# wouter-rombouts/fast-losless-image-compression-format

Hardware: AMD Instinct MI355X
Metric: encode+decode MPixels/s on 4K RGBA at 1/2/4/8 MI355X; bitstream bit-exact (higher is better)
Workload: dtype u8

## Files before the change

### fast-losless-image-compression-format_amd/csrc/nice_dec_rec.hpp

```cpp
#pragma once
#include <hip/hip_runtime.h>
#include <stdint.h>

#include "nice_format.h"

namespace nice {

__device__ __forceinline__ void set_status(int32_t* st, int32_t code) {
  atomicCAS(reinterpret_cast<int*>(st), 0, code);
}

constexpr uint32_t REC_RUN = 1u << 28;
constexpr uint32_t REC_K = 0xFFu | (0xFFu << 10) | (0xFFu << 20);
constexpr uint32_t REC_TAG_MASK = (3u << 8) | (3u << 18);
__device__ __forceinline__ uint32_t rec_tagbits(uint32_t tag) { return ((tag & 3u) << 8) | ((tag >> 2) << 18); }
__device__ __forceinline__ uint32_t rec_canon(uint32_t r, uint32_t tag) {
  return (r & REC_TAG_MASK) == rec_tagbits(tag) ? r : REC_RUN;
}
__device__ __forceinline__ uint32_t rec_cls(uint32_t r) { return r >> 28; }
__device__ __forceinline__ uint32_t rec_c(uint32_t r) { return r & REC_K; }
__device__ __forceinline__ uint32_t rec_spread(uint32_t v) {
  return (v & 0xFFu) | ((v & 0xFF00u) << 2) | ((v & 0xFF0000u) << 4);
}
__host__ __device__ constexpr int cls_rows(int c) {
  return c < 4 ? 0 : c == 4 ? 1 : c == 5 ? 1 : c == 6 ? 2 : c == 7 ? 1 : c <= 10 ? 3 : c == 11 ? 1 : c <= 13 ? 3 : 0;
}
__host__ __device__ constexpr int cls_px(int c) {
  return c < 4 ? c : c == 4 ? 0 : c == 5 ? -1 : c == 6 ? 0 : c == 7 ? -3 : c == 8 ? -1 : c == 9 ? 0
       : c == 10 ? 1 : c == 11 ? 3 : c == 12 ? 3 : c == 13 ? -3 : 0;
}
__host__ __device__ constexpr int id_cls(int id) {
  return id == 0 ? 1 : id == 1 ? 4 : id == 2 ? 5 : id == 3 ? 2 : id == 4 ? 6
       : id == 5 ? 1 : id == 6 ? 4 : id == 7 ? 5 : id == 8 ? 7 : id == 9 ? 3 : id == 10 ? 8
       : id == 11 ? 9 : id == 12 ? 10 : id == 13 ? 11 : id == 14 ? 12 : 13;
}
__host__ __device__ constexpr bool cls_table_ok() {
  for (int id = 0; id < 16; ++id) {
    const int rows = id < 5 ? br_rows(id) : lr_rows(id - 5), px = id < 5 ? br_px(id) : lr_px(id - 5);
    if (cls_rows(id_cls(id)) != rows || cls_px(id_cls(id)) != px) return false;
  }
  return true;
}
static_assert(cls_table_ok(), "reference offsets (code.rs:141-145) map onto the record classes");
constexpr unsigned long long ID_CLS_PACK = [] {
  unsigned long long v = 0;
  for (int id = 0; id < 16; ++id) v |= (unsigned long long)id_cls(id) << (4 * id);
  return v;
}();
constexpr uint32_t CLS_ROWS_PACK = [] {
  uint32_t v = 0;
  for (int c = 0; c < 16; ++c) v |= (uint32_t)cls_rows(c) << (2 * c);
  return v;
}();
constexpr unsigned long long CLS_PX_PACK = [] {
  unsigned long long v = 0;
  for (int c = 0; c < 16; ++c) v |= (unsigned long long)(cls_px(c) + 3) << (3 * c);
  return v;
}();

}
```

### fast-losless-image-compression-format_amd/csrc/nice_decode.hip

```cpp
#include <hip/hip_runtime.h>
#include <stdint.h>

#include <type_traits>

#include "../../include/nice.h"
#include "nice_bits.hpp"
#include "nice_dec_rec.hpp"
#include "nice_format.h"
#include "nice_kernels.h"

namespace nice {

__device__ __forceinline__ uint32_t n_chunks(uint64_t len, uint64_t D, uint32_t cb) {
  const uint64_t bits = len * 8;
  return bits > D ? (uint32_t)((bits - D + cb - 1) / cb) : 0u;
}

__global__ __launch_bounds__(256) void dec_tables(DecArgs a) {
  __shared__ uint8_t lens[N_BINS];
  __shared__ uint8_t smax[N_STREAMS];
  __shared__ uint16_t order[N_BINS];
  __shared__ int bad;
  const uint32_t f = blockIdx.x;
  const uint64_t len = a.stream_len[f];
// ... 277 lines not shown
  uint4 pp[8];
};

__device__ inline void load_lut(LutLds& S, const DecTables* T) {
  const uint4* s = reinterpret_cast<const uint4*>(T->lut);
  uint4* d = reinterpret_cast<uint4*>(S.lut);
  for (uint32_t i = threadIdx.x; i < sizeof(S.lut) / 16; i += blockDim.x) d[i] = s[i];
  for (uint32_t i = threadIdx.x; i < N_BINS; i += blockDim.x) {
    S.lo[i] = T->lo[i];
    S.sym[i] = T->sym[i];
    S.len[i] = T->len[i];
  }
  if (threadIdx.x < N_STREAMS) {
    const int st = (int)threadIdx.x;
    S.gp[st] = (uint32_t)T->lut_off[st] | ((uint32_t)T->lut_bits[st] << 16) | ((uint32_t)T->max_aob[st] << 24);
    S.gs[st] = (uint32_t)stream_base(st) | ((uint32_t)stream_size(st) << 16);
  }
  if (threadIdx.x < 8u) {
    const uint32_t m = threadIdx.x;
    uint32_t w[4];
#pragma unroll
    for (uint32_t i = 0; i < 4; ++i) {
      const uint32_t st = m < 5u ? pay_stream(m, i) : 0u;
      w[i] = (32u - T->lut_bits[st]) | ((uint32_t)T->lut_off[st] << 17);
    }
    S.pp[m] = make_uint4(w[0], w[1], w[2], w[3]);
  }
}

__device__ __forceinline__ uint32_t stream_word(const uint8_t* p, uint64_t len, uint32_t w) {
  uint32_t v = 0;
  for (int k = 0; k < 4; ++k) {
    const uint64_t i = (uint64_t)w * 4 + k;
    v = (v << 8) | (i < len ? p[i] : (len ? p[len - 1] : 0u));
  }
  return v;
}

struct Lane {
  unsigned long long pos;
  unsigned long long win;
  uint32_t avail;
  uint32_t rp;
  uint32_t ws;
};
__device__ __forceinline__ bool lane_ok(const Lane& L) { return L.rp + PIXEL_WORDS <= RING_W; }

// ... 122 lines not shown
__device__ __forceinline__ uint32_t pixel_event_fast(Lane& L, const uint32_t* my, const LutLds& S,
                                                     const StreamParams& G, uint32_t& s0, uint32_t& s1,
                                                     uint32_t& s2, uint32_t& s3) {
  const uint32_t o = (uint32_t)(L.pos >> 5) - L.ws;
  const uint32_t sh = (uint32_t)L.pos & 31u;
  const uint32_t w0 = my[o], w1 = my[o + 1], w2 = my[o + 2];
  unsigned long long win = ((((unsigned long long)w0 << 32) | w1) << sh) | (((unsigned long long)w2 << sh) >> 32);
  uint32_t tot = 0;
  const uint32_t pfx = fsym(win, tot, S, G.g[PFX_STREAM]);
  if (pfx < (uint32_t)P_RUN1) {
    const bool rgb = pfx == (uint32_t)P_RGB, lu = pfx == (uint32_t)P_LUMA, l2 = pfx == (uint32_t)P_LUMA2;
    const uint4 pp = S.pp[pfx];
    s0 = fsym(win, tot, S, pp.x);
    if (rgb || lu || l2) {
      s1 = fsym(win, tot, S, pp.y);
      s2 = fsym(win, tot, S, pp.z);
      if (lu) s3 = fsym(win, tot, S, pp.w);
    }
  }
  L.pos += tot;
  return pfx;
}

__device__ __forceinline__ uint32_t pixel_event_fast_at(const uint32_t* my, const LutLds& S, uint32_t fp_pfx,
                                                        uint32_t o, uint32_t sh, uint32_t& s0, uint32_t& s1,
                                                        uint32_t& s2, uint32_t& s3, uint32_t& tot) {
  const uint32_t w0 = my[o], w1 = my[o + 1], w2 = my[o + 2];
  unsigned long long win = ((((unsigned long long)w0 << 32) | w1) << sh) | (((unsigned long long)w2 << sh) >> 32);
  tot = 0;
  const uint32_t pfx = fsym(win, tot, S, fp_pfx);
  if (pfx < (uint32_t)P_RUN1) {
    const bool rgb = pfx == (uint32_t)P_RGB, lu = pfx == (uint32_t)P_LUMA, l2 = pfx == (uint32_t)P_LUMA2;
    const uint4 pp = S.pp[pfx];
    s0 = fsym(win, tot, S, pp.x);
    if (rgb || lu || l2) {
      s1 = fsym(win, tot, S, pp.y);
      s2 = fsym(win, tot, S, pp.z);
      if (lu) s3 = fsym(win, tot, S, pp.w);
    }
  }
  return pfx;
}

__device__ __forceinline__ uint32_t pixel_count(uint32_t pfx, uint32_t& dk) {
  if (pfx < (uint32_t)P_RUN1) { dk = 0; return 1u; }
  const uint32_t sh = (3u * dk) & 63u;
  const uint64_t c = ((uint64_t)(pfx - P_RUN1) << sh) + (dk == 0 ? 1u : 0u);
  dk = dk >= 64u ? 1u : dk + 1u;
  return c > 0xFFFFFFFFull ? 0xFFFFFFFFu : (uint32_t)c;
}
__device__ __forceinline__ uint32_t sat_add(uint32_t a, uint32_t b) { return a + b < a ? 0xFFFFFFFFu : a + b; }

constexpr unsigned long long PS_MASK = (1ull << 51) - 1ull;
__device__ __forceinline__ unsigned long long ps_pack(unsigned long long rel, uint32_t dk) {
  return rel | ((unsigned long long)dk << 44);
}


__global__ __launch_bounds__(256) void dec_init_entries(DecArgs a) {
  const uint32_t f = blockIdx.y;
  for (uint32_t j = blockIdx.x * 256 + threadIdx.x; j < a.max_chunks; j += gridDim.x * 256) {
// ... 13 lines not shown

constexpr uint32_t SLICE_EMIT = 0, SLICE_HEAD_EMIT = 1, SLICE_PLACE = 2;
__device__ __forceinline__ uint32_t slice_route(const DecArgs& a, uint64_t base, uint32_t j, uint32_t& ag,
                                                uint32_t& nvalid, uint32_t& hn) {
  const unsigned long long last = a.last[base + j];
  ag = a.agree[base + j];
  const uint32_t nev = a.ev_n[base + j];
  unsigned long long e = 0;
  uint32_t hev_n = EV_OVERFLOW, hev_ag = AGREE_NONE;
  if (a.hev) {
    e = j == 0 ? 0ull : a.entry[base + j];
    hev_n = a.hev_n[base + j];
    hev_ag = a.hev_ag[base + j];
  }
  nvalid = (uint32_t)(last >> 56);
  hn = 0;
  if (ag == AGREE_NONE || nev == EV_OVERFLOW || ag > nvalid) return SLICE_EMIT;
  if (ag == 0u) return SLICE_PLACE;
  if ((last & PS_MASK) != e || hev_n == EV_OVERFLOW || hev_ag != ag) return SLICE_HEAD_EMIT;
  hn = hev_n;
  return SLICE_PLACE;
}

__device__ __forceinline__ uint32_t ev_pack(uint32_t pfx, uint32_t s0, uint32_t s1, uint32_t s2, uint32_t s3) {
  return pfx | (s0 << 3) | (s1 << 12) | (s2 << 20) | (pfx == (uint32_t)P_LUMA ? s3 << 7 : 0u);
}

__global__ __launch_bounds__(DEC_PARSE_THREADS) PARSE_ATTR void dec_sync(DecArgs a, uint32_t* changed, const uint32_t* prev,
                                                              uint32_t* fchanged) {
  __shared__ LutLds S;
  __shared__ __attribute__((aligned(16))) uint32_t ring[DEC_PARSE_THREADS * RING_STRIDE];
  if (prev && *prev == 0) return;
  const uint32_t f = blockIdx.x / a.chunk_blocks;
  const uint32_t jb = blockIdx.x % a.chunk_blocks;
  if (a.status[f] != 0) return;
  const uint64_t len = a.stream_len[f];
  const uint64_t D = a.data_start[f];
  const uint32_t nc = n_chunks(len, D, a.chunk_bits);
  if (jb * DEC_PARSE_THREADS >= nc) return;
  const uint32_t j = jb * DEC_PARSE_THREADS + threadIdx.x;
  const uint64_t base = (uint64_t)f * a.max_chunks;
  unsigned long long e = 0, last = ~0ull;
  if (j < nc) {
    e = j == 0 ? 0ull : a.entry[base + j];
    last = a.last[base + j];
  }
  const bool need = j < nc && (last == ~0ull || (last & PS_MASK) != e);
  if (!__syncthreads_or(need)) return;
  load_lut(S, reinterpret_cast<const DecTables*>(a.tables) + f);
// ... 100 lines not shown
      constexpr bool HEAD = decltype(keep_tag)::value == 2;
      if (active && (r >= rlim || px > N)) active = false;
      if (active && r >= nck) {
        const uint32_t cur = (r - b31) | (dk << 20);
        if (check && k < nvalid_old && (uint32_t)ck_old == cur) {
          synced = true;
          active = false;
        } else {
          ck[(uint64_t)k * a.max_chunks] = cur | ((unsigned long long)px << 32);
          if (keep) evck[(uint64_t)k * a.max_chunks] = ne;
          ++k;
          nck = k < a.n_ck ? nck + a.ck_bits : 0xFFFFFFFFu;
          ck_old = (check && k < nvalid_old) ? ck[(uint64_t)k * a.max_chunks] : ~0ull;
        }
      }
      if ((!(KEEP || HEAD) || SLOT == 0) && !__any(active)) return false;
      if (__any(active && r >= rfill)) {
        const uint32_t wsa = (bwl + (r >> 5)) & ~3u;
        ring_fill_ws(wring, p, len, al16, wsa);
        wsr = wsa - bwl;
        rfill = (wsr + RING_W - 2u) << 5;
      }
      if (active) {
        uint32_t s0 = 0, s1 = 0, s2 = 0, s3 = 0, tot;
        const uint32_t pfx = pixel_event_fast_at(my, S, fp_pfx, (r >> 5) - wsr, r & 31u, s0, s1, s2, s3, tot);
        r += tot;
        uint32_t c;
        if (pfx < (uint32_t)P_RUN1) {
          dk = 0;
          c = 1u;
        } else {
          const uint32_t sh = (3u * dk) & 63u, d = pfx - (uint32_t)P_RUN1;
          if (sh < 30u) {
            c = (d << sh) + (dk == 0 ? 1u : 0u);
          } else {
            const uint64_t c64 = (uint64_t)d << sh;
            c = c64 > 0xFFFFFFFFull ? 0xFFFFFFFFu : (uint32_t)c64;
          }
          dk = dk >= 64u ? 1u : dk + 1u;
        }
        px = sat_add(px, c);
        if (KEEP && keep) {
          const uint32_t ev = pfx < (uint32_t)P_RUN1 ? ev_pack(pfx, s0, s1, s2, s3) : EV_RUN | min(c, EV_RUN - 1u);
          if constexpr (SLOT == 0) q0 = ev;
          if constexpr (SLOT == 1) q1 = ev;
          if constexpr (SLOT == 2) q2 = ev;
          if constexpr (SLOT == 3) {
            q3 = ev;
            if (ne < a.ev_cap) *reinterpret_cast<uint4*>(evp + ev_word(ne - 3u)) = make_uint4(q0, q1, q2, q3);
          }
          ++ne;
        }
        if (HEAD && hkeep) {
          const uint32_t ev = pfx < (uint32_t)P_RUN1 ? ev_pack(pfx, s0, s1, s2, s3) : EV_RUN | min(c, EV_RUN - 1u);
          if constexpr (SLOT == 0) q0 = ev;
          if constexpr (SLOT == 1) q1 = ev;
          if constexpr (SLOT == 2) q2 = ev;
          if constexpr (SLOT == 3) {
            q3 = ev;
            if (ne < a.hev_cap) *reinterpret_cast<uint4*>(evp + ev_word(ne - 3u)) = make_uint4(q0, q1, q2, q3);
          }
          ++ne;
        }
      }
      return true;
    };
    using keep_none = std::integral_constant<int, 0>;
    using keep_first = std::integral_constant<int, 1>;
    using keep_head = std::integral_constant<int, 2>;
    if (__any(keep && active)) {
      for (;;) {
        if (!step(std::integral_constant<int, 0>{}, keep_first{})) break;
        if (!step(std::integral_constant<int, 1>{}, keep_first{})) break;
        if (!step(std::integral_constant<int, 2>{}, keep_first{})) break;
        if (!step(std::integral_constant<int, 3>{}, keep_first{})) break;
      }
    } else if (__any(hkeep && active)) {
// ... 288 lines not shown
      if (dk != 0 && pfx == (uint32_t)P_RUN1) (void)pixel_count(pfx, dk);
      else active = false;
      continue;
    }
    if (pfx < (uint32_t)P_RUN1) {
      (void)rd(pay_stream(pfx, 0));
      if (pfx == (uint32_t)P_RGB || pfx == (uint32_t)P_LUMA || pfx == (uint32_t)P_LUMA2) {
        (void)rd(pay_stream(pfx, 1));
        (void)rd(pay_stream(pfx, 2));
        if (pfx == (uint32_t)P_LUMA) (void)rd(S_LUMA_OTHER);
      }
      q += 1;
      dk = 0;
      closed = false;
    } else {
      q += pixel_count(pfx, dk);
      closed = closed || q == N;
    }
  }
  if (hang) set_status(&a.status[f], NICE_E_UNSUPPORTED);
}


__device__ __forceinline__ uint32_t make_event_rec(uint64_t W, uint32_t mode, uint32_t s0, uint32_t s1,
                                                   uint32_t s2, uint32_t s3) {
  const bool isbr = mode == P_BACK_REF, islu = mode == P_LUMA;
  const bool issd = mode == P_SMALL_DIFF, isl2 = mode == P_LUMA2;
  const uint32_t id = min(isbr ? s0 : 5u + s0, 15u);
  const uint32_t cls = (uint32_t)(ID_CLS_PACK >> (4 * id)) & 15u;
  const uint64_t rows = (CLS_ROWS_PACK >> (2 * cls)) & 3u;
  const int64_t off = (int64_t)(rows * W) + (int64_t)((CLS_PX_PACK >> (3 * cls)) & 7u) - 3;
  const bool bad0 = (isbr && s0 >= 5u) || (islu && s0 >= 11u) || off < 0;
  const uint32_t gl = (s1 - 32u) & 255u;
  const uint32_t c_lu = ((s2 - 16u + gl) & 255u) | (gl << 10) | (((s3 - 16u + gl) & 255u) << 20);
  const uint32_t rd = s0 % 7u, t1 = s0 / 7u;
  const uint32_t c_sd = ((rd - 3u) & 255u) | ((((t1 % 7u) - 3u) & 255u) << 10) | ((((t1 / 7u) - 3u) & 255u) << 20);
  const uint32_t g2 = (s0 - 32u) & 255u;
  const uint32_t c_l2 = ((s1 - 16u + g2) & 255u) | (g2 << 10) | (((s2 - 16u + g2) & 255u) << 20);
  const uint32_t c_rgb = (s0 & 255u) | ((s1 & 255u) << 10) | ((s2 & 255u) << 20);
  const uint32_t r = (isbr || islu) ? ((cls << 28) | (islu ? c_lu : 0u)) : issd ? c_sd : isl2 ? c_l2 : c_rgb;
  return r | (isl2 ? EV_L2 : 0u) | ((isbr || islu) && bad0 ? EV_BAD : 0u);
}
__device__ __forceinline__ bool rec_bad_at(uint32_t ev, uint64_t q, uint64_t W) {
  const uint32_t cls = rec_cls(ev);
  const uint64_t rows = (CLS_ROWS_PACK >> (2 * cls)) & 3u;
  const uint64_t off = rows * W + ((CLS_PX_PACK >> (3 * cls)) & 7u) - 3u;
  return (ev & EV_BAD) || ((ev & EV_L2) ? q < W : (cls != 0u && q < off));
}
__device__ __forceinline__ uint32_t make_record(uint64_t W, uint64_t q, uint32_t mode, uint32_t s0,
                                                uint32_t s1, uint32_t s2, uint32_t s3, bool& bad) {
  const uint32_t ev = make_event_rec(W, mode, s0, s1, s2, s3);
  bad = rec_bad_at(ev, q, W);
  return ev & ~(EV_L2 | EV_BAD);
}

struct RecGroup {
  unsigned long long grp;
  uint32_t v0, v1, v2, v3, mask;
  __device__ __forceinline__ void flush(uint32_t* rec, unsigned long long lo, unsigned long long hi) {
    if (!mask) return;
    if (grp >= lo && grp + 4 <= hi) {
      uint4* dst = reinterpret_cast<uint4*>(__builtin_assume_aligned(rec + grp, 16));
      *dst = make_uint4(v0, v1, v2, v3);
    } else {
      if (mask & 1u) rec[grp] = v0;
      if (mask & 2u) rec[grp + 1] = v1;
      if (mask & 4u) rec[grp + 2] = v2;
      if (mask & 8u) rec[grp + 3] = v3;
    }
  }
  __device__ __forceinline__ void put(uint32_t* rec, unsigned long long lo, unsigned long long cur,
                                      uint32_t r) {
    const unsigned long long g4 = cur & ~3ull;
    if (g4 != grp) {
      flush(rec, lo, cur);
      grp = g4;
      v0 = v1 = v2 = v3 = REC_RUN;
// ... 179 lines not shown
    if (route == SLICE_EMIT) return min(subs, 1u + nvalid / step);
    if (route == SLICE_PLACE) return 0u;
    return (ag + step - 1) / step;
  };
  uint32_t cnt = 0;
  for (uint32_t j = c0; j < c1; ++j) cnt += nsub(j);
  part[threadIdx.x] = cnt;
  __syncthreads();
  for (uint32_t d = 1; d < 1024; d <<= 1) {
    const uint32_t t = threadIdx.x >= d ? part[threadIdx.x - d] : 0u;
    __syncthreads();
    part[threadIdx.x] += t;
    __syncthreads();
  }
  uint32_t o = part[threadIdx.x] - cnt;
  uint32_t* items = a.head_items + base * subs;
  for (uint32_t j = c0; j < c1; ++j) {
    const uint32_t n = nsub(j);
    for (uint32_t s = 0; s < n; ++s) items[o++] = j * subs + s;
  }
  if (threadIdx.x == 1023) a.head_count[f] = part[1023];
}

__device__ __forceinline__ uint32_t place_record(uint32_t ev, uint32_t q, uint32_t W, const uint32_t* sdl,
                                                 const uint2* idt, bool& bad) {
  const uint32_t pfx = ev & 7u;
  const uint32_t pm = 1u << pfx;
  const bool isbr = (pm & (1u << P_BACK_REF)) != 0u, islu = (pm & (1u << P_LUMA)) != 0u;
  const bool issd = (pm & (1u << P_SMALL_DIFF)) != 0u, isl2 = (pm & (1u << P_LUMA2)) != 0u;
  const uint32_t s0 = (ev >> 3) & 511u, s1 = (ev >> 12) & 255u, s2 = (ev >> 20) & 255u, s3 = (ev >> 7) & 31u;
  const uint32_t s0l = s0 & 15u;
  const uint32_t id = min(isbr ? s0 : 5u + s0l, 15u);
  const uint2 ct = idt[id];
  const uint32_t cls = ct.x, off3 = ct.y;
  const bool bad_ref = (isbr && s0 >= 5u) || (islu && s0l >= 11u) || off3 < 3u || q + 3u < off3;
  const uint32_t gl = (s1 - 32u) & 255u;
  const uint32_t c_lu = ((s2 - 16u + gl) & 255u) | (gl << 10) | (((s3 - 16u + gl) & 255u) << 20);
  const uint32_t c_sd = sdl[min(s0, 342u)];
  const uint32_t g2 = (s0 - 32u) & 255u;
  const uint32_t c_l2 = ((s1 - 16u + g2) & 255u) | (g2 << 10) | (((s2 - 16u + g2) & 255u) << 20);
  uint32_t c_rgb = (s0 & 255u) | (s1 << 10) | (s2 << 20);
  bad = (isbr || islu) ? bad_ref : (isl2 && q < W);
  uint32_t c_br = (cls << 28) | (islu ? c_lu : 0u);
  uint32_t c_sd2 = c_sd, c_l22 = c_l2;
  asm volatile("" : "+v"(c_br), "+v"(c_sd2), "+v"(c_l22), "+v"(c_rgb));
  return (isbr || islu) ? c_br : issd ? c_sd2 : isl2 ? c_l22 : c_rgb;
}

struct alignas(16) SdlTable {
  uint32_t v[344];
};
constexpr SdlTable make_sdl_table() {
  SdlTable t{};
  for (uint32_t i = 0; i < 343u; ++i) {
    const uint32_t rd = i % 7u, t1 = i / 7u;
    t.v[i] = ((rd - 3u) & 255u) | ((((t1 % 7u) - 3u) & 255u) << 10) | ((((t1 / 7u) - 3u) & 255u) << 20);
  }
  return t;
}
__device__ __constant__ SdlTable kSdl = make_sdl_table();

__global__ __launch_bounds__(64 * DEC_PLACE_WAVES) void dec_place(DecArgs a) {
  __shared__ __attribute__((aligned(16))) uint32_t sdl[344];
  __shared__ uint2 idt[16];
  if (threadIdx.x < 16u) {
    const uint32_t id = threadIdx.x;
    const uint32_t cls = (uint32_t)(ID_CLS_PACK >> (4u * id)) & 15u;
    idt[id] = make_uint2(cls, (uint32_t)((CLS_ROWS_PACK >> (2u * cls)) & 3u) * a.W +
                                  (uint32_t)((CLS_PX_PACK >> (3u * cls)) & 7u));
  }
  if (threadIdx.x < 86u)
    reinterpret_cast<uint4*>(sdl)[threadIdx.x] = reinterpret_cast<const uint4*>(kSdl.v)[threadIdx.x];
  __syncthreads();
  const uint32_t lane = threadIdx.x & 63u;
  const uint32_t nbx = gridDim.x, nwg = nbx * gridDim.y, lin = blockIdx.y * nbx + blockIdx.x;
  const uint32_t xq = nwg / 8u, xr = nwg % 8u, xcd = lin % 8u;
  const uint32_t lg = (xcd < xr ? xcd * (xq + 1u) : xr * (xq + 1u) + (xcd - xr) * xq) + lin / 8u;
  const uint32_t f = lg / nbx, j = (lg % nbx) * DEC_PLACE_WAVES + (uint32_t)__builtin_amdgcn_readfirstlane((int)(threadIdx.x >> 6));
  if (a.status[f] != 0) return;
  const uint64_t len = a.stream_len[f];
  const uint64_t D = a.data_start[f];
  if (j >= n_chunks(len, D, a.chunk_bits)) return;
  const uint64_t base = (uint64_t)f * a.max_chunks;
  uint32_t ag, nvalid, hn;
  const uint32_t route = slice_route(a, base, j, ag, nvalid, hn);
  const uint32_t nev = a.ev_n[base + j];
  if (a.stats && lane == 0) {
    const uint32_t b = nev == EV_OVERFLOW ? 7u : ag == AGREE_NONE ? 6u : ag == 0u ? 0u : ag == 1u ? 1u
                     : ag <= 4u ? 2u : ag <= 16u ? 3u : ag <= 64u ? 4u : 5u;
    atomicAdd(&a.stats[50 + b], 1ull);
    atomicAdd(&a.stats[route == SLICE_EMIT ? 29 : route == SLICE_HEAD_EMIT ? 28 : ag == 0u ? 26 : 27], 1ull);
  }
  if (route == SLICE_EMIT) return;
  const bool head = route == SLICE_PLACE && ag != 0u;
  const uint64_t cki = (uint64_t)f * a.n_ck * a.max_chunks + j + (uint64_t)(ag ? ag - 1u : 0u) * a.max_chunks;
  auto uni = [](uint32_t v) { return (uint32_t)__builtin_amdgcn_readfirstlane((int)v); };
  const uint32_t i_first1 = uni(ag == 0u ? 0u : a.ev_ck[cki]), nev1 = uni(nev);
  hn = uni(hn);
  const unsigned long long q_first = a.chunk_start[base + j];
  const unsigned long long q_meet_v = q_first + (ag == 0u ? 0ull : (a.ck[cki] >> 32));
  const unsigned long long q_meet = ((unsigned long long)uni((uint32_t)(q_meet_v >> 32)) << 32) | uni((uint32_t)q_meet_v);
  unsigned long long q = head ? q_first : q_meet;
  const uint64_t N = (uint64_t)a.W * a.H;
  if (q > N) return;
  uint32_t* rec = a.recs + (uint64_t)f * a.rec_stride;
  const bool strict = (a.flags & NICE_DEC_STRICT_REFERENCE) != 0;
  bool err = false, stopped = false;
  for (uint32_t part = head ? 0u : 1u; part < 2u && !stopped; ++part) {
  const uint32_t* evp = part == 0u ? a.hev + hev_group(a, f, j) : a.ev + ev_group(a, f, j);
  const uint32_t i_first = part == 0u ? 0u : i_first1, nev = part == 0u ? hn : nev1;
  if (part == 1u && head && q != q_meet) {
    if (lane == 0) {
      if (a.stats) atomicAdd(&a.stats[30], 1ull);
      set_status(&a.status[f], NICE_E_HIP);
    }
    return;
  }
  if (i_first >= nev) continue;
  const uint32_t ev_last = nev - 1u;
  uint32_t nx[4];
#pragma unroll
  for (int k = 0; k < 4; ++k) nx[k] = evp[ev_word(min(i_first + 64u * k + lane, ev_last))];
  for (uint32_t i = i_first; i < nev; i += 256u) {
    uint32_t ev[4], r[4];
#pragma unroll
    for (int k = 0; k < 4; ++k) {
      ev[k] = nx[k];
      nx[k] = evp[ev_word(min(i + 256u + 64u * k + lane, ev_last))];
    }
    {
      const uint32_t N32 = (uint32_t)N;
      uint32_t c32[4];
      bool big = false;
#pragma unroll
      for (int k = 0; k < 4; ++k) {
        const bool valid = i + 64u * k + lane < nev;
        c32[k] = valid ? ((ev[k] & EV_RUN) ? (ev[k] & ~EV_RUN) : 1u) : 0u;
        big = big || c32[k] >= 65536u;
      }
      if (!__any(big)) {
        uint32_t qb[4];
        uint32_t base = (uint32_t)q;
        bool stop = false;
#pragma unroll
        for (int k = 0; k < 4; ++k) {
          if (i + 64u * k >= nev) break;
          const bool valid = i + 64u * k + lane < nev;
          const bool run = (ev[k] & EV_RUN) != 0u;
          const uint32_t incl = wave_incl_scan(c32[k]);
          qb[k] = base + incl - c32[k];
          base += (uint32_t)__builtin_amdgcn_readlane((int)incl, 63);
          bool rbad = false;
          r[k] = place_record(ev[k], min(qb[k], N32), a.W, sdl, idt, rbad);
          stop = stop || (valid && (qb[k] >= N32 || (run ? qb[k] + c32[k] > N32 : rbad)));
        }
        if (!__any(stop)) {
#pragma unroll
          for (int k = 0; k < 4; ++k) {
            if (i + 64u * k >= nev) break;
            if (i + 64u * k + lane < nev && !(ev[k] & EV_RUN)) rec[qb[k]] = r[k] | rec_tagbits(a.rec_tag);
          }
          q = base;
          continue;
        }
      }
    }
    unsigned long long c[4], qk[4], carry = 0;
    uint32_t stop_k = 4u, stop_lane = 64u;
    bool stop_at_n = false, stop_run = false;
#pragma unroll
    for (int k = 0; k < 4; ++k) {
      const uint32_t x = i + 64u * k + lane;
      const bool valid = x < nev;
      const bool run = (ev[k] & EV_RUN) != 0u;
      c[k] = valid ? (run ? (ev[k] & ~EV_RUN) : 1u) : 0u;
      unsigned long long incl;
      if (!__any(c[k] >= (1u << 25))) {
        incl = wave_incl_scan((uint32_t)c[k]);
      } else {
        incl = c[k];
#pragma unroll
        for (int o = 1; o < 64; o <<= 1) {
          const unsigned long long t = __shfl_up(incl, o);
          if ((int)lane >= o) incl += t;
        }
      }
      const unsigned long long qb = q + carry + incl - c[k];
      carry += __shfl(incl, 63);
      qk[k] = qb;
      bool rbad = false;
      r[k] = place_record(ev[k], (uint32_t)min(qb, N), a.W, sdl, idt, rbad);
      const bool at_n = valid && qb == N && !(run && c[k] == 0);
      const bool bad = valid && !at_n && (run ? qb + c[k] > N : rbad);
      const unsigned long long m = __ballot(at_n || bad);
      if (stop_k == 4u && m) {
        stop_k = (uint32_t)k;
        stop_lane = (uint32_t)__builtin_ctzll(m);
        stop_at_n = __shfl(at_n ? 1 : 0, (int)stop_lane) != 0;
        stop_run = __shfl(run ? 1 : 0, (int)stop_lane) != 0;
      }
    }
#pragma unroll
    for (int k = 0; k < 4; ++k) {
      const bool keep = (uint32_t)k < stop_k || ((uint32_t)k == stop_k && lane < stop_lane);
      if (keep && i + 64u * k + lane < nev && !(ev[k] & EV_RUN)) rec[qk[k]] = r[k] | rec_tagbits(a.rec_tag);
    }
    if (stop_k < 4u) {
      if (lane == 0) err = stop_at_n ? (strict && stop_run) : true;
      stopped = true;
      break;
    }
    q += carry;
  }
  }
// ... 6 lines not shown
```

### fast-losless-image-compression-format_amd/csrc/nice_kernels.h

```cpp
#pragma once
#include <hip/hip_runtime.h>
#include <stdint.h>

#include "nice_geom.h"

namespace nice {

constexpr uint32_t FLAG_LONG = 1u;
constexpr uint32_t FLAG_BAD = 2u;

struct EncArgs {
  const uint8_t* px;
  uint64_t frame_stride;
  uint32_t n_frames, W, H, C;
  uint8_t channels_out;
  uint32_t tiles_per_frame, tiles_per_block;
  uint8_t* out;
  uint64_t out_stride;
  unsigned long long* out_len;
  uint32_t* hist;
  uint32_t* tile_first;
  uint32_t* tile_last;
  uint32_t* tile_next;
  uint32_t* cmask;
// ... 114 lines not shown
  uint32_t* ev_n;
  uint32_t* agree;
  uint32_t* head_items;
  uint32_t* head_count;
  uint32_t* hev;
  uint32_t hev_cap;
  uint32_t* hev_n;
  uint32_t* hev_ag;
  uint32_t strips;
  unsigned long long* hand;
  uint32_t* hand_abort;
  uint32_t split_f0;
  uint32_t redo;
  uint32_t test_absent_strip;
  uint32_t flow_k, flow_ring;
  const uint32_t* unsettled;
  const unsigned long long* stream_off;
  uint64_t packed_bytes;
};
__device__ __forceinline__ const uint8_t* dec_stream_ptr(const DecArgs& a, uint32_t f) {
  return a.streams + (a.stream_off ? (uint64_t)a.stream_off[f] : (uint64_t)f * a.stream_stride);
}
constexpr uint32_t SPLIT_ABORT_ERR = 1u, SPLIT_REDO = 2u;
constexpr uint32_t EV_RUN = 1u << 31, EV_BAD = 1u << 9, EV_L2 = 1u << 8;
constexpr uint32_t EV_OVERFLOW = 0xFFFFFFFFu, AGREE_NONE = 0xFFFFu;

__global__ void dec_tables(DecArgs a);
__global__ void dec_init_entries(DecArgs a);
__global__ void dec_sync(DecArgs a, uint32_t* changed, const uint32_t* prev, uint32_t* fchanged);
__global__ void dec_sync_settle(DecArgs a, const uint32_t* last_changed, const uint32_t* fchanged, uint32_t* settled);
__global__ void dec_scan(DecArgs a);
__global__ void dec_strict_refill(DecArgs a);
__global__ void dec_emit(DecArgs a);
__global__ void dec_place(DecArgs a);
__global__ void dec_heads(DecArgs a);
__global__ void dec_reconstruct(DecArgs a);
__global__ void dec_rows(DecArgs a);
__global__ void dec_rows_wide(DecArgs a);
__global__ void dec_rows8(DecArgs a);
__global__ void dec_rows_flow(DecArgs a);
__global__ void dec_rows_split(DecArgs a);

__device__ __forceinline__ uint32_t wave_incl_scan(uint32_t v) {
  v += (uint32_t)__builtin_amdgcn_update_dpp(0, (int)v, 0x111, 0xF, 0xF, false);
  v += (uint32_t)__builtin_amdgcn_update_dpp(0, (int)v, 0x112, 0xF, 0xF, false);
  v += (uint32_t)__builtin_amdgcn_update_dpp(0, (int)v, 0x114, 0xF, 0xF, false);
  v += (uint32_t)__builtin_amdgcn_update_dpp(0, (int)v, 0x118, 0xF, 0xF, false);
// ... 14 lines not shown
```

Before: 69290.

## Repack decode events so placement becomes table-driven masked ORs

Changes the event word layout so each decoded symbol is shifted into its final record bit position during parsing, using shifts stored in the per-prefix LUT entry. Placement then builds a record from a 128-entry shared table of class/mask entries plus a small-diff lookup, replacing per-event branch-heavy reconstruction. A deep-region fast path skips the per-event reference bounds check once the position is at least three rows in. This cuts ALU work in dec_place at the cost of larger shared tables and a new event encoding shared between parse and place, which must stay consistent.

```diff
diff --git a/fast-losless-image-compression-format_amd/csrc/nice_dec_event.hpp b/fast-losless-image-compression-format_amd/csrc/nice_dec_event.hpp
--- /dev/null
+++ b/fast-losless-image-compression-format_amd/csrc/nice_dec_event.hpp
@@ -0,0 +1,164 @@
+#pragma once
+#include <stdint.h>
+
+#include "nice_format.h"
+
+#ifndef NICE_HDI
+#if defined(__HIPCC__) || defined(__CUDACC__)
+#define NICE_HDI __host__ __device__ __forceinline__
+#else
+#define NICE_HDI inline
+#endif
+#endif
+
+namespace nice {
+
+constexpr uint32_t REC_RUN = 1u << 28;
+constexpr uint32_t REC_K = 0xFFu | (0xFFu << 10) | (0xFFu << 20);
+constexpr uint32_t REC_TAG_MASK = (3u << 8) | (3u << 18);
+NICE_HDI uint32_t rec_tagbits(uint32_t tag) { return ((tag & 3u) << 8) | ((tag >> 2) << 18); }
+NICE_HDI uint32_t rec_canon(uint32_t r, uint32_t tag) {
+  return (r & REC_TAG_MASK) == rec_tagbits(tag) ? r : REC_RUN;
+}
+NICE_HDI uint32_t rec_cls(uint32_t r) { return r >> 28; }
+NICE_HDI uint32_t rec_c(uint32_t r) { return r & REC_K; }
+NICE_HDI uint32_t rec_spread(uint32_t v) {
+  return (v & 0xFFu) | ((v & 0xFF00u) << 2) | ((v & 0xFF0000u) << 4);
+}
+NICE_HD constexpr int cls_rows(int c) {
+  return c < 4 ? 0 : c == 4 ? 1 : c == 5 ? 1 : c == 6 ? 2 : c == 7 ? 1 : c <= 10 ? 3 : c == 11 ? 1 : c <= 13 ? 3 : 0;
+}
+NICE_HD constexpr int cls_px(int c) {
+  return c < 4 ? c : c == 4 ? 0 : c == 5 ? -1 : c == 6 ? 0 : c == 7 ? -3 : c == 8 ? -1 : c == 9 ? 0
+       : c == 10 ? 1 : c == 11 ? 3 : c == 12 ? 3 : c == 13 ? -3 : 0;
+}
+NICE_HD constexpr int id_cls(int id) {
+  return id == 0 ? 1 : id == 1 ? 4 : id == 2 ? 5 : id == 3 ? 2 : id == 4 ? 6
+       : id == 5 ? 1 : id == 6 ? 4 : id == 7 ? 5 : id == 8 ? 7 : id == 9 ? 3 : id == 10 ? 8
+       : id == 11 ? 9 : id == 12 ? 10 : id == 13 ? 11 : id == 14 ? 12 : 13;
+}
+NICE_HD constexpr bool cls_table_ok() {
+  for (int id = 0; id < 16; ++id) {
+    const int rows = id < 5 ? br_rows(id) : lr_rows(id - 5), px = id < 5 ? br_px(id) : lr_px(id - 5);
+    if (cls_rows(id_cls(id)) != rows || cls_px(id_cls(id)) != px) return false;
+  }
+  return true;
+}
+static_assert(cls_table_ok(), "reference offsets (code.rs:141-145) map onto the record classes");
+constexpr unsigned long long ID_CLS_PACK = [] {
+  unsigned long long v = 0;
+  for (int id = 0; id < 16; ++id) v |= (unsigned long long)id_cls(id) << (4 * id);
+  return v;
+}();
+constexpr uint32_t CLS_ROWS_PACK = [] {
+  uint32_t v = 0;
+  for (int c = 0; c < 16; ++c) v |= (uint32_t)cls_rows(c) << (2 * c);
+  return v;
+}();
+constexpr unsigned long long CLS_PX_PACK = [] {
+  unsigned long long v = 0;
+  for (int c = 0; c < 16; ++c) v |= (unsigned long long)(cls_px(c) + 3) << (3 * c);
+  return v;
+}();
+
+constexpr uint32_t EV_BAD = 1u << 9, EV_L2 = 1u << 8;
+
+NICE_HDI uint32_t make_event_rec(uint64_t W, uint32_t mode, uint32_t s0, uint32_t s1, uint32_t s2, uint32_t s3) {
+  const bool isbr = mode == P_BACK_REF, islu = mode == P_LUMA;
+  const bool issd = mode == P_SMALL_DIFF, isl2 = mode == P_LUMA2;
+  const uint32_t idr = isbr ? s0 : 5u + s0;
+  const uint32_t id = idr < 15u ? idr : 15u;
+  const uint32_t cls = (uint32_t)(ID_CLS_PACK >> (4 * id)) & 15u;
+  const uint64_t rows = (CLS_ROWS_PACK >> (2 * cls)) & 3u;
+  const int64_t off = (int64_t)(rows * W) + (int64_t)((CLS_PX_PACK >> (3 * cls)) & 7u) - 3;
+  const bool bad0 = (isbr && s0 >= 5u) || (islu && s0 >= 11u) || off < 0;
+  const uint32_t gl = (s1 - 32u) & 255u;
+  const uint32_t c_lu = ((s2 - 16u + gl) & 255u) | (gl << 10) | (((s3 - 16u + gl) & 255u) << 20);
+  const uint32_t rd = s0 % 7u, t1 = s0 / 7u;
+  const uint32_t c_sd = ((rd - 3u) & 255u) | ((((t1 % 7u) - 3u) & 255u) << 10) | ((((t1 / 7u) - 3u) & 255u) << 20);
+  const uint32_t g2 = (s0 - 32u) & 255u;
+  const uint32_t c_l2 = ((s1 - 16u + g2) & 255u) | (g2 << 10) | (((s2 - 16u + g2) & 255u) << 20);
+  const uint32_t c_rgb = (s0 & 255u) | ((s1 & 255u) << 10) | ((s2 & 255u) << 20);
+  const uint32_t r = (isbr || islu) ? ((cls << 28) | (islu ? c_lu : 0u)) : issd ? c_sd : isl2 ? c_l2 : c_rgb;
+  return r | (isl2 ? EV_L2 : 0u) | ((isbr || islu) && bad0 ? EV_BAD : 0u);
+}
+NICE_HDI bool rec_bad_at(uint32_t ev, uint64_t q, uint64_t W) {
+  const uint32_t cls = rec_cls(ev);
+  const uint64_t rows = (CLS_ROWS_PACK >> (2 * cls)) & 3u;
+  const uint64_t off = rows * W + ((CLS_PX_PACK >> (3 * cls)) & 7u) - 3u;
+  return (ev & EV_BAD) || ((ev & EV_L2) ? q < W : (cls != 0u && q < off));
+}
+NICE_HDI uint32_t make_record(uint64_t W, uint64_t q, uint32_t mode, uint32_t s0, uint32_t s1, uint32_t s2,
+                              uint32_t s3, bool& bad) {
+  const uint32_t ev = make_event_rec(W, mode, s0, s1, s2, s3);
+  bad = rec_bad_at(ev, q, W);
+  return ev & ~(EV_L2 | EV_BAD);
+}
+
+constexpr uint32_t EV_RUN = 1u << 31;
+constexpr uint32_t EV_PFX_SHIFT = 28, EV_ID_SHIFT = 16;
+NICE_HD constexpr uint32_t ev_shift(uint32_t pfx, uint32_t i) {
+  return pfx == (uint32_t)P_BACK_REF ? (i == 0 ? EV_ID_SHIFT : 0u)
+       : pfx == (uint32_t)P_RGB ? (i == 0 ? 0u : i == 1 ? 10u : i == 2 ? 20u : 0u)
+       : pfx == (uint32_t)P_LUMA ? (i == 0 ? EV_ID_SHIFT : i == 1 ? 10u : i == 2 ? 0u : 20u)
+       : pfx == (uint32_t)P_LUMA2 ? (i == 0 ? 10u : i == 1 ? 0u : i == 2 ? 20u : 0u)
+       : 0u;
+}
+NICE_HDI uint32_t ev_pack(uint32_t pfx, uint32_t s0, uint32_t s1, uint32_t s2, uint32_t s3) {
+  return (pfx << EV_PFX_SHIFT) | (s0 << ev_shift(pfx, 0)) | (s1 << ev_shift(pfx, 1)) | (s2 << ev_shift(pfx, 2)) |
+         (s3 << ev_shift(pfx, 3));
+}
+
+struct alignas(16) PlaceEnt {
+  uint32_t cls, ml, mr, msd;
+};
+constexpr uint32_t PLACE_ENTRIES = 128;
+NICE_HDI PlaceEnt place_entry(uint32_t entry, uint32_t W, uint32_t& off3) {
+  const uint32_t pfx = entry & 7u, idf = entry >> 3;
+  const bool isbr = pfx == (uint32_t)P_BACK_REF, islu = pfx == (uint32_t)P_LUMA;
+  const bool isl2 = pfx == (uint32_t)P_LUMA2;
+  const uint32_t idr = isbr ? idf : 5u + idf;
+  const uint32_t id = idr < 15u ? idr : 15u;
+  const uint32_t cls = (uint32_t)(ID_CLS_PACK >> (4u * id)) & 15u;
+  const uint32_t o3 = (uint32_t)((CLS_ROWS_PACK >> (2u * cls)) & 3u) * W + (uint32_t)((CLS_PX_PACK >> (3u * cls)) & 7u);
+  const bool rejected = (isbr && idf >= 5u) || (islu && idf >= 11u) || o3 < 3u;
+  const bool isref = isbr || islu;
+  off3 = isref ? (rejected ? 0xFFFFFFFFu : o3) : isl2 ? W + 3u : 0u;
+  PlaceEnt e;
+  e.cls = isref ? cls << 28 : 0u;
+  e.ml = (islu || isl2) ? REC_K : 0u;
+  e.mr = pfx == (uint32_t)P_RGB ? REC_K : (isref && rejected) ? EV_BAD : 0u;
+  e.msd = pfx == (uint32_t)P_SMALL_DIFF ? 511u : 0u;
+  return e;
+}
+struct alignas(16) SdlTable {
+  uint32_t v[344];
+};
+constexpr SdlTable make_sdl_table() {
+  SdlTable t{};
+  for (uint32_t i = 0; i < 343u; ++i) {
+    const uint32_t rd = i % 7u, t1 = i / 7u;
+    t.v[i] = ((rd - 3u) & 255u) | ((((t1 % 7u) - 3u) & 255u) << 10) | ((((t1 / 7u) - 3u) & 255u) << 20);
+  }
+  return t;
+}
+
+constexpr uint32_t EV_LUMA_MASK = 0xFFu | (0x3Fu << 10) | (0xFFu << 20);
+constexpr uint32_t EV_LUMA_K = 240u | (224u << 10) | (240u << 20);
+
+NICE_HDI bool place_deep(uint64_t q0, uint64_t W) { return q0 >= 3u * W + 3u; }
+
+template <bool CHECK>
+NICE_HDI uint32_t place_record(uint32_t ev, uint32_t q, const uint32_t* sdl, const PlaceEnt* idt,
+                               const uint32_t* off3, bool& bad) {
+  const uint32_t entry = ((ev >> (EV_ID_SHIFT - 3u)) & 0x78u) | (ev >> EV_PFX_SHIFT);
+  const PlaceEnt t = idt[entry];
+  const uint32_t c_sd = sdl[(ev & t.msd) | (343u & ~t.msd)];
+  const uint32_t lt = (ev & EV_LUMA_MASK) + EV_LUMA_K;
+  const uint32_t x = lt + ((lt >> 10) & 255u) * 0x100001u;
+  if (CHECK) bad = q + 3u < off3[entry];
+  else bad = t.mr == EV_BAD;
+  return t.cls | (x & t.ml) | (ev & t.mr) | c_sd;
+}
+
+}
diff --git a/fast-losless-image-compression-format_amd/csrc/nice_dec_rec.hpp b/fast-losless-image-compression-format_amd/csrc/nice_dec_rec.hpp
--- a/fast-losless-image-compression-format_amd/csrc/nice_dec_rec.hpp
+++ b/fast-losless-image-compression-format_amd/csrc/nice_dec_rec.hpp
@@ -2,6 +2,7 @@
 #include <hip/hip_runtime.h>
 #include <stdint.h>
 
+#include "nice_dec_event.hpp"
 #include "nice_format.h"
 
 namespace nice {
@@ -10,52 +11,4 @@
   atomicCAS(reinterpret_cast<int*>(st), 0, code);
 }
 
-constexpr uint32_t REC_RUN = 1u << 28;
-constexpr uint32_t REC_K = 0xFFu | (0xFFu << 10) | (0xFFu << 20);
-constexpr uint32_t REC_TAG_MASK = (3u << 8) | (3u << 18);
-__device__ __forceinline__ uint32_t rec_tagbits(uint32_t tag) { return ((tag & 3u) << 8) | ((tag >> 2) << 18); }
-__device__ __forceinline__ uint32_t rec_canon(uint32_t r, uint32_t tag) {
-  return (r & REC_TAG_MASK) == rec_tagbits(tag) ? r : REC_RUN;
 }
-__device__ __forceinline__ uint32_t rec_cls(uint32_t r) { return r >> 28; }
-__device__ __forceinline__ uint32_t rec_c(uint32_t r) { return r & REC_K; }
-__device__ __forceinline__ uint32_t rec_spread(uint32_t v) {
-  return (v & 0xFFu) | ((v & 0xFF00u) << 2) | ((v & 0xFF0000u) << 4);
-}
-__host__ __device__ constexpr int cls_rows(int c) {
-  return c < 4 ? 0 : c == 4 ? 1 : c == 5 ? 1 : c == 6 ? 2 : c == 7 ? 1 : c <= 10 ? 3 : c == 11 ? 1 : c <= 13 ? 3 : 0;
-}
-__host__ __device__ constexpr int cls_px(int c) {
-  return c < 4 ? c : c == 4 ? 0 : c == 5 ? -1 : c == 6 ? 0 : c == 7 ? -3 : c == 8 ? -1 : c == 9 ? 0
-       : c == 10 ? 1 : c == 11 ? 3 : c == 12 ? 3 : c == 13 ? -3 : 0;
-}
-__host__ __device__ constexpr int id_cls(int id) {
-  return id == 0 ? 1 : id == 1 ? 4 : id == 2 ? 5 : id == 3 ? 2 : id == 4 ? 6
-       : id == 5 ? 1 : id == 6 ? 4 : id == 7 ? 5 : id == 8 ? 7 : id == 9 ? 3 : id == 10 ? 8
-       : id == 11 ? 9 : id == 12 ? 10 : id == 13 ? 11 : id == 14 ? 12 : 13;
-}
-__host__ __device__ constexpr bool cls_table_ok() {
-  for (int id = 0; id < 16; ++id) {
-    const int rows = id < 5 ? br_rows(id) : lr_rows(id - 5), px = id < 5 ? br_px(id) : lr_px(id - 5);
-    if (cls_rows(id_cls(id)) != rows || cls_px(id_cls(id)) != px) return false;
-  }
-  return true;
-}
-static_assert(cls_table_ok(), "reference offsets (code.rs:141-145) map onto the record classes");
-constexpr unsigned long long ID_CLS_PACK = [] {
-  unsigned long long v = 0;
-  for (int id = 0; id < 16; ++id) v |= (unsigned long long)id_cls(id) << (4 * id);
-  return v;
-}();
-constexpr uint32_t CLS_ROWS_PACK = [] {
-  uint32_t v = 0;
-  for (int c = 0; c < 16; ++c) v |= (uint32_t)cls_rows(c) << (2 * c);
-  return v;
-}();
-constexpr unsigned long long CLS_PX_PACK = [] {
-  unsigned long long v = 0;
-  for (int c = 0; c < 16; ++c) v |= (unsigned long long)(cls_px(c) + 3) << (3 * c);
-  return v;
-}();
-
-}
diff --git a/fast-losless-image-compression-format_amd/csrc/nice_decode.hip b/fast-losless-image-compression-format_amd/csrc/nice_decode.hip
--- a/fast-losless-image-compression-format_amd/csrc/nice_decode.hip
+++ b/fast-losless-image-compression-format_amd/csrc/nice_decode.hip
@@ -323,7 +323,7 @@
 #pragma unroll
     for (uint32_t i = 0; i < 4; ++i) {
       const uint32_t st = m < 5u ? pay_stream(m, i) : 0u;
-      w[i] = (32u - T->lut_bits[st]) | ((uint32_t)T->lut_off[st] << 17);
+      w[i] = (32u - T->lut_bits[st]) | (ev_shift(m, i) << 5) | ((uint32_t)T->lut_off[st] << 17);
     }
     S.pp[m] = make_uint4(w[0], w[1], w[2], w[3]);
   }
@@ -492,9 +492,11 @@
   return pfx;
 }
 
+template <bool EV = false>
 __device__ __forceinline__ uint32_t pixel_event_fast_at(const uint32_t* my, const LutLds& S, uint32_t fp_pfx,
                                                         uint32_t o, uint32_t sh, uint32_t& s0, uint32_t& s1,
-                                                        uint32_t& s2, uint32_t& s3, uint32_t& tot) {
+                                                        uint32_t& s2, uint32_t& s3, uint32_t& tot,
+                                                        uint32_t* evw = nullptr) {
   const uint32_t w0 = my[o], w1 = my[o + 1], w2 = my[o + 2];
   unsigned long long win = ((((unsigned long long)w0 << 32) | w1) << sh) | (((unsigned long long)w2 << sh) >> 32);
   tot = 0;
@@ -503,10 +505,15 @@
     const bool rgb = pfx == (uint32_t)P_RGB, lu = pfx == (uint32_t)P_LUMA, l2 = pfx == (uint32_t)P_LUMA2;
     const uint4 pp = S.pp[pfx];
     s0 = fsym(win, tot, S, pp.x);
+    if constexpr (EV) *evw = (pfx << EV_PFX_SHIFT) | (s0 << ((pp.x >> 5) & 31u));
     if (rgb || lu || l2) {
       s1 = fsym(win, tot, S, pp.y);
       s2 = fsym(win, tot, S, pp.z);
-      if (lu) s3 = fsym(win, tot, S, pp.w);
+      if constexpr (EV) *evw |= (s1 << ((pp.y >> 5) & 31u)) | (s2 << ((pp.z >> 5) & 31u));
+      if (lu) {
+        s3 = fsym(win, tot, S, pp.w);
+        if constexpr (EV) *evw |= s3 << ((pp.w >> 5) & 31u);
+      }
     }
   }
   return pfx;
@@ -566,9 +573,6 @@
   return SLICE_PLACE;
 }
 
-__device__ __forceinline__ uint32_t ev_pack(uint32_t pfx, uint32_t s0, uint32_t s1, uint32_t s2, uint32_t s3) {
-  return pfx | (s0 << 3) | (s1 << 12) | (s2 << 20) | (pfx == (uint32_t)P_LUMA ? s3 << 7 : 0u);
-}
 
 __global__ __launch_bounds__(DEC_PARSE_THREADS) PARSE_ATTR void dec_sync(DecArgs a, uint32_t* changed, const uint32_t* prev,
                                                               uint32_t* fchanged) {
@@ -715,8 +719,9 @@
         rfill = (wsr + RING_W - 2u) << 5;
       }
       if (active) {
-        uint32_t s0 = 0, s1 = 0, s2 = 0, s3 = 0, tot;
-        const uint32_t pfx = pixel_event_fast_at(my, S, fp_pfx, (r >> 5) - wsr, r & 31u, s0, s1, s2, s3, tot);
+        uint32_t s0 = 0, s1 = 0, s2 = 0, s3 = 0, tot, evw = 0;
+        const uint32_t pfx = pixel_event_fast_at<KEEP || HEAD>(my, S, fp_pfx, (r >> 5) - wsr, r & 31u, s0, s1, s2,
+                                                               s3, tot, &evw);
         r += tot;
         uint32_t c;
         if (pfx < (uint32_t)P_RUN1) {
@@ -734,7 +739,7 @@
         }
         px = sat_add(px, c);
         if (KEEP && keep) {
-          const uint32_t ev = pfx < (uint32_t)P_RUN1 ? ev_pack(pfx, s0, s1, s2, s3) : EV_RUN | min(c, EV_RUN - 1u);
+          const uint32_t ev = pfx < (uint32_t)P_RUN1 ? evw : EV_RUN | min(c, EV_RUN - 1u);
           if constexpr (SLOT == 0) q0 = ev;
           if constexpr (SLOT == 1) q1 = ev;
           if constexpr (SLOT == 2) q2 = ev;
@@ -745,7 +750,7 @@
           ++ne;
         }
         if (HEAD && hkeep) {
-          const uint32_t ev = pfx < (uint32_t)P_RUN1 ? ev_pack(pfx, s0, s1, s2, s3) : EV_RUN | min(c, EV_RUN - 1u);
+          const uint32_t ev = pfx < (uint32_t)P_RUN1 ? evw : EV_RUN | min(c, EV_RUN - 1u);
           if constexpr (SLOT == 0) q0 = ev;
           if constexpr (SLOT == 1) q1 = ev;
           if constexpr (SLOT == 2) q2 = ev;
@@ -1080,37 +1085,6 @@
 }
 
 
-__device__ __forceinline__ uint32_t make_event_rec(uint64_t W, uint32_t mode, uint32_t s0, uint32_t s1,
-                                                   uint32_t s2, uint32_t s3) {
-  const bool isbr = mode == P_BACK_REF, islu = mode == P_LUMA;
-  const bool issd = mode == P_SMALL_DIFF, isl2 = mode == P_LUMA2;
-  const uint32_t id = min(isbr ? s0 : 5u + s0, 15u);
-  const uint32_t cls = (uint32_t)(ID_CLS_PACK >> (4 * id)) & 15u;
-  const uint64_t rows = (CLS_ROWS_PACK >> (2 * cls)) & 3u;
-  const int64_t off = (int64_t)(rows * W) + (int64_t)((CLS_PX_PACK >> (3 * cls)) & 7u) - 3;
-  const bool bad0 = (isbr && s0 >= 5u) || (islu && s0 >= 11u) || off < 0;
-  const uint32_t gl = (s1 - 32u) & 255u;
-  const uint32_t c_lu = ((s2 - 16u + gl) & 255u) | (gl << 10) | (((s3 - 16u + gl) & 255u) << 20);
-  const uint32_t rd = s0 % 7u, t1 = s0 / 7u;
-  const uint32_t c_sd = ((rd - 3u) & 255u) | ((((t1 % 7u) - 3u) & 255u) << 10) | ((((t1 / 7u) - 3u) & 255u) << 20);
-  const uint32_t g2 = (s0 - 32u) & 255u;
-  const uint32_t c_l2 = ((s1 - 16u + g2) & 255u) | (g2 << 10) | (((s2 - 16u + g2) & 255u) << 20);
-  const uint32_t c_rgb = (s0 & 255u) | ((s1 & 255u) << 10) | ((s2 & 255u) << 20);
-  const uint32_t r = (isbr || islu) ? ((cls << 28) | (islu ? c_lu : 0u)) : issd ? c_sd : isl2 ? c_l2 : c_rgb;
-  return r | (isl2 ? EV_L2 : 0u) | ((isbr || islu) && bad0 ? EV_BAD : 0u);
-}
-__device__ __forceinline__ bool rec_bad_at(uint32_t ev, uint64_t q, uint64_t W) {
-  const uint32_t cls = rec_cls(ev);
-  const uint64_t rows = (CLS_ROWS_PACK >> (2 * cls)) & 3u;
-  const uint64_t off = rows * W + ((CLS_PX_PACK >> (3 * cls)) & 7u) - 3u;
-  return (ev & EV_BAD) || ((ev & EV_L2) ? q < W : (cls != 0u && q < off));
-}
-__device__ __forceinline__ uint32_t make_record(uint64_t W, uint64_t q, uint32_t mode, uint32_t s0,
-                                                uint32_t s1, uint32_t s2, uint32_t s3, bool& bad) {
-  const uint32_t ev = make_event_rec(W, mode, s0, s1, s2, s3);
-  bad = rec_bad_at(ev, q, W);
-  return ev & ~(EV_L2 | EV_BAD);
-}
 
 struct RecGroup {
   unsigned long long grp;
@@ -1336,55 +1310,23 @@
   if (threadIdx.x == 1023) a.head_count[f] = part[1023];
 }
 
-__device__ __forceinline__ uint32_t place_record(uint32_t ev, uint32_t q, uint32_t W, const uint32_t* sdl,
-                                                 const uint2* idt, bool& bad) {
-  const uint32_t pfx = ev & 7u;
-  const uint32_t pm = 1u << pfx;
-  const bool isbr = (pm & (1u << P_BACK_REF)) != 0u, islu = (pm & (1u << P_LUMA)) != 0u;
-  const bool issd = (pm & (1u << P_SMALL_DIFF)) != 0u, isl2 = (pm & (1u << P_LUMA2)) != 0u;
-  const uint32_t s0 = (ev >> 3) & 511u, s1 = (ev >> 12) & 255u, s2 = (ev >> 20) & 255u, s3 = (ev >> 7) & 31u;
-  const uint32_t s0l = s0 & 15u;
-  const uint32_t id = min(isbr ? s0 : 5u + s0l, 15u);
-  const uint2 ct = idt[id];
-  const uint32_t cls = ct.x, off3 = ct.y;
-  const bool bad_ref = (isbr && s0 >= 5u) || (islu && s0l >= 11u) || off3 < 3u || q + 3u < off3;
-  const uint32_t gl = (s1 - 32u) & 255u;
-  const uint32_t c_lu = ((s2 - 16u + gl) & 255u) | (gl << 10) | (((s3 - 16u + gl) & 255u) << 20);
-  const uint32_t c_sd = sdl[min(s0, 342u)];
-  const uint32_t g2 = (s0 - 32u) & 255u;
-  const uint32_t c_l2 = ((s1 - 16u + g2) & 255u) | (g2 << 10) | (((s2 - 16u + g2) & 255u) << 20);
-  uint32_t c_rgb = (s0 & 255u) | (s1 << 10) | (s2 << 20);
-  bad = (isbr || islu) ? bad_ref : (isl2 && q < W);
-  uint32_t c_br = (cls << 28) | (islu ? c_lu : 0u);
-  uint32_t c_sd2 = c_sd, c_l22 = c_l2;
-  asm volatile("" : "+v"(c_br), "+v"(c_sd2), "+v"(c_l22), "+v"(c_rgb));
-  return (isbr || islu) ? c_br : issd ? c_sd2 : isl2 ? c_l22 : c_rgb;
-}
-
-struct alignas(16) SdlTable {
-  uint32_t v[344];
-};
-constexpr SdlTable make_sdl_table() {
-  SdlTable t{};
-  for (uint32_t i = 0; i < 343u; ++i) {
-    const uint32_t rd = i % 7u, t1 = i / 7u;
-    t.v[i] = ((rd - 3u) & 255u) | ((((t1 % 7u) - 3u) & 255u) << 10) | ((((t1 / 7u) - 3u) & 255u) << 20);
-  }
-  return t;
-}
 __device__ __constant__ SdlTable kSdl = make_sdl_table();
 
 __global__ __launch_bounds__(64 * DEC_PLACE_WAVES) void dec_place(DecArgs a) {
-  __shared__ __attribute__((aligned(16))) uint32_t sdl[344];
-  __shared__ uint2 idt[16];
-  if (threadIdx.x < 16u) {
-    const uint32_t id = threadIdx.x;
-    const uint32_t cls = (uint32_t)(ID_CLS_PACK >> (4u * id)) & 15u;
-    idt[id] = make_uint2(cls, (uint32_t)((CLS_ROWS_PACK >> (2u * cls)) & 3u) * a.W +
-                                  (uint32_t)((CLS_PX_PACK >> (3u * cls)) & 7u));
+  __shared__ __attribute__((aligned(16))) uint32_t sdl[512];
+  __shared__ PlaceEnt idt[PLACE_ENTRIES];
+  __shared__ uint32_t off3[PLACE_ENTRIES];
+  static_assert(64 * DEC_PLACE_WAVES >= PLACE_ENTRIES + 128, "one thread per table entry");
+  if (threadIdx.x >= 64u * DEC_PLACE_WAVES - PLACE_ENTRIES) {
+    const uint32_t entry = threadIdx.x - (64u * DEC_PLACE_WAVES - PLACE_ENTRIES);
+    uint32_t o3;
+    idt[entry] = place_entry(entry, a.W, o3);
+    off3[entry] = o3;
   }
   if (threadIdx.x < 86u)
     reinterpret_cast<uint4*>(sdl)[threadIdx.x] = reinterpret_cast<const uint4*>(kSdl.v)[threadIdx.x];
+  else if (threadIdx.x < 128u)
+    reinterpret_cast<uint4*>(sdl)[threadIdx.x] = make_uint4(0u, 0u, 0u, 0u);
   __syncthreads();
   const uint32_t lane = threadIdx.x & 63u;
   const uint32_t nbx = gridDim.x, nwg = nbx * gridDim.y, lin = blockIdx.y * nbx + blockIdx.x;
@@ -1417,6 +1359,7 @@
   unsigned long long q = head ? q_first : q_meet;
   const uint64_t N = (uint64_t)a.W * a.H;
   if (q > N) return;
+  const uint32_t deep32 = 3ull * a.W + 3u > 0xFFFFFFFFull ? 0xFFFFFFFFu : 3u * a.W + 3u;
   uint32_t* rec = a.recs + (uint64_t)f * a.rec_stride;
   const bool strict = (a.flags & NICE_DEC_STRICT_REFERENCE) != 0;
   bool err = false, stopped = false;
@@ -1444,6 +1387,7 @@
     }
     {
       const uint32_t N32 = (uint32_t)N;
+      const bool deep = uni((uint32_t)q) >= deep32;
       uint32_t c32[4];
       bool big = false;
 #pragma unroll
@@ -1456,18 +1400,23 @@
         uint32_t qb[4];
         uint32_t base = (uint32_t)q;
         bool stop = false;
-#pragma unroll
-        for (int k = 0; k < 4; ++k) {
-          if (i + 64u * k >= nev) break;
-          const bool valid = i + 64u * k + lane < nev;
-          const bool run = (ev[k] & EV_RUN) != 0u;
-          const uint32_t incl = wave_incl_scan(c32[k]);
-          qb[k] = base + incl - c32[k];
-          base += (uint32_t)__builtin_amdgcn_readlane((int)incl, 63);
-          bool rbad = false;
-          r[k] = place_record(ev[k], min(qb[k], N32), a.W, sdl, idt, rbad);
-          stop = stop || (valid && (qb[k] >= N32 || (run ? qb[k] + c32[k] > N32 : rbad)));
-        }
+        auto rows = [&](auto check_tag) {
+          constexpr bool CHECK = decltype(check_tag)::value;
+#pragma unroll
+          for (int k = 0; k < 4; ++k) {
+            if (i + 64u * k >= nev) break;
+            const bool valid = i + 64u * k + lane < nev;
+            const bool run = (ev[k] & EV_RUN) != 0u;
+            const uint32_t incl = wave_incl_scan(c32[k]);
+            qb[k] = base + incl - c32[k];
+            base += (uint32_t)__builtin_amdgcn_readlane((int)incl, 63);
+            bool rbad = false;
+            r[k] = place_record<CHECK>(ev[k], min(qb[k], N32), sdl, idt, off3, rbad);
+            stop = stop || (valid && (qb[k] >= N32 || (run ? qb[k] + c32[k] > N32 : rbad)));
+          }
+        };
+        if (deep) rows(std::false_type{});
+        else rows(std::true_type{});
         if (!__any(stop)) {
 #pragma unroll
           for (int k = 0; k < 4; ++k) {
@@ -1503,7 +1452,7 @@
       carry += __shfl(incl, 63);
       qk[k] = qb;
       bool rbad = false;
-      r[k] = place_record(ev[k], (uint32_t)min(qb, N), a.W, sdl, idt, rbad);
+      r[k] = place_record<true>(ev[k], (uint32_t)min(qb, N), sdl, idt, off3, rbad);
       const bool at_n = valid && qb == N && !(run && c[k] == 0);
       const bool bad = valid && !at_n && (run ? qb + c[k] > N : rbad);
       const unsigned long long m = __ballot(at_n || bad);
diff --git a/fast-losless-image-compression-format_amd/csrc/nice_kernels.h b/fast-losless-image-compression-format_amd/csrc/nice_kernels.h
--- a/fast-losless-image-compression-format_amd/csrc/nice_kernels.h
+++ b/fast-losless-image-compression-format_amd/csrc/nice_kernels.h
@@ -160,7 +160,6 @@
   return a.streams + (a.stream_off ? (uint64_t)a.stream_off[f] : (uint64_t)f * a.stream_stride);
 }
 constexpr uint32_t SPLIT_ABORT_ERR = 1u, SPLIT_REDO = 2u;
-constexpr uint32_t EV_RUN = 1u << 31, EV_BAD = 1u << 9, EV_L2 = 1u << 8;
 constexpr uint32_t EV_OVERFLOW = 0xFFFFFFFFu, AGREE_NONE = 0xFFFFu;
 
 __global__ void dec_tables(DecArgs a);
```

Result: faster. 70700, median of 6 (+2.0%).
